# gevaertlab/RNA-GAN

Hardware: AMD Instinct MI355X
Metric: training imgs/sec (G+D WGAN-GP step, 256x256) (higher is better)
Workload: dtype bf16; 1 GPU; RNA-GAN lung (betaVAE-conditioned wganvae path) 256x256, DCGAN enc2048/step64, per-GPU batch 64, one iteration = G-loss + D-loss + GP steps; global_batch=64, parallelism=dp1, ranks=1, rna_features=19198, hip_graphs=True, dp_statistics=rank-local (DDP)

## Files before the change

rna_gan_amd/csrc/rg_api.hip:

```cpp
#include "rg_common.h"
#include "rg_internal.h"
#include <stdarg.h>
#include <stdio.h>
#include <stdlib.h>
#include <string.h>
#include <ctype.h>

static thread_local char g_err[512] = "";

void rg_set_error(const char* fmt, ...) {
  va_list ap;
  va_start(ap, fmt);
  vsnprintf(g_err, sizeof(g_err), fmt, ap);
  va_end(ap);
}

extern "C" int rg_version(void) { return 618; }
extern "C" const char* rg_last_error(void) { return g_err; }

static const char* const g_opt_names[] = {"conv8", "conv8_blocks", "conv_tile", "xcd", "class_fast", "wgrad_blocks",
                                          "wgrad8", "conv_v1", "stream_tile", "narrow8", "conv8_mfma", "conv8_epi", "wgrad8_blocks", "korder", "convp", "convp_blocks",
                                          "fp8_mx", "wgrad8n", "f32mma", "convd", "convd_blocks", "skinny128", "slab16", "wslab16", "bn_rev", "wgrad8_mfma", "narrow32", "upimg", "upimg_blocks"};
constexpr int G_NOPT = sizeof(g_opt_names) / sizeof(g_opt_names[0]);
static int g_opt_override[G_NOPT];
static int g_opt_env[G_NOPT];

int rg_option(const char* name, int dflt) {
  for (int i = 0; i < G_NOPT; ++i) {
    if (strcmp(name, g_opt_names[i]) != 0) continue;
    if (g_opt_override[i] > 0) return g_opt_override[i] - 1;
    if (g_opt_env[i] == 0) {
      char var[64] = "RNAGAN_";
      size_t n = strlen(var);
      for (const char* c = name; *c && n + 1 < sizeof(var); ++c) var[n++] = (char)toupper((unsigned char)*c);
      var[n] = 0;
      const char* e = getenv(var);
      g_opt_env[i] = e ? atoi(e) + 1 : -1;
      if (g_opt_env[i] == 0) g_opt_env[i] = -1;
    }
    return g_opt_env[i] > 0 ? g_opt_env[i] - 1 : dflt;
  }
  return dflt;
}

extern "C" int rg_set_option(const char* name, int value) {
  RG_REQUIRE(name, RG_EINVAL, "set_option: null name");
  for (int i = 0; i < G_NOPT; ++i)
    if (strcmp(name, g_opt_names[i]) == 0) { g_opt_override[i] = value < 0 ? 0 : value + 1; return RG_OK; }
  rg_set_error("set_option: unknown option '%s'", name);
  return RG_EINVAL;
}

static bool want_mfma(int algo, int dtype) { return algo != RG_ALGO_GENERIC && dtype == RG_H16; }

extern "C" int rg_pack_conv_weight(const float* w, void* wdn, void* wup, int O, int I, int dtype, void* stream) {
  RG_REQUIRE(w && O > 0 && I > 0, RG_EINVAL, "pack_conv_weight: bad args");
  RG_REQUIRE(dtype == RG_H16, RG_EUNSUPPORTED, "pack_conv_weight: only bf16 packs exist (fp32 kernels read w)");
  return rg_mfma_pack_conv_weight(w, wdn, wup, O, I, rg_stream(stream));
}

static bool conv_planned(int up, int N, int Hlow, int Wlow, int O, int I, int dtype, int algo) {
  return N > 0 && Hlow > 0 && Wlow > 0 && O > 0 && I > 0 && want_mfma(algo, dtype) &&
         rg_mfma_conv_supported(N, Hlow, Wlow, up ? O : I, up ? I : O);
}
extern "C" size_t rg_conv_workspace_bytes(int up, int N, int Hlow, int Wlow, int O, int I, int dtype, int algo) {
  return conv_planned(up, N, Hlow, Wlow, O, I, dtype, algo) ? rg_mfma_conv_plan(up, N, Hlow, Wlow, O, I).ws_bytes : 0;
}
extern "C" int rg_conv_stats_rows(int up, int N, int Hlow, int Wlow, int O, int I, int dtype, int algo) {
  return conv_planned(up, N, Hlow, Wlow, O, I, dtype, algo) ? rg_mfma_conv_plan(up, N, Hlow, Wlow, O, I).stats_rows : 0;
}
extern "C" int rg_conv_split(int up, int N, int Hlow, int Wlow, int O, int I, int dtype, int algo) {
  return conv_planned(up, N, Hlow, Wlow, O, I, dtype, algo) ? rg_mfma_conv_plan(up, N, Hlow, Wlow, O, I).nsplit : 1;
}
extern "C" int rg_conv_slab_dtype(int up, int N, int Hlow, int Wlow, int O, int I, int dtype, int algo) {
  return conv_planned(up, N, Hlow, Wlow, O, I, dtype, algo) && rg_mfma_conv_plan(up, N, Hlow, Wlow, O, I).slab16 ? RG_H16 : RG_F32;
}

extern "C" int rg_conv_down_partial(const void* x, const void* wdn, int N, int Hi, int Wi, int I, int O, int dtype, int algo,
                                    void* ws, size_t ws_bytes, void* stream) {
  RG_REQUIRE(x && wdn && ws && N > 0 && Hi > 0 && Wi > 0 && I > 0 && O > 0 && Hi % 2 == 0 && Wi % 2 == 0, RG_EINVAL,
             "conv_down_partial: bad args");
  RG_REQUIRE(rg_conv_split(0, N, Hi / 2, Wi / 2, O, I, dtype, algo) > 1, RG_EUNSUPPORTED,
             "conv_down_partial: this shape does not run split-K (rg_conv_split)");
  return rg_mfma_conv_down(x, wdn, nullptr, N, Hi, Wi, I, O, nullptr, ws, ws_bytes, rg_stream(stream), 1);
}

extern "C" int rg_conv_up_partial(const void* x, const void* wup, int N, int Ho, int Wo, int O, int I, int dtype, int algo,
                                  void* ws, size_t ws_bytes, void* stream) {
  RG_REQUIRE(x && wup && ws && N > 0 && Ho > 0 && Wo > 0 && I > 0 && O > 0, RG_EINVAL, "conv_up_partial: bad args");
  RG_REQUIRE(rg_conv_split(1, N, Ho, Wo, O, I, dtype, algo) > 1, RG_EUNSUPPORTED,
             "conv_up_partial: this shape does not run split-K (rg_conv_split)");
  return rg_mfma_conv_up(x, wup, nullptr, N, Ho, Wo, O, I, nullptr, 1.f, nullptr, ws, ws_bytes, rg_stream(stream), nullptr,
                         nullptr, 1.f, 0, 1);
}

extern "C" int rg_conv_down(const void* x, const float* w, const void* wdn, void* y, int N, int Hi, int Wi, int I,
                            int O, float* stats_partial, int dtype, int algo, void* ws, size_t ws_bytes, void* stream) {
  RG_REQUIRE(x && y && N > 0 && Hi > 0 && Wi > 0 && I > 0 && O > 0 && Hi % 2 == 0 && Wi % 2 == 0, RG_EINVAL,
             "conv_down: bad args");
  if (want_mfma(algo, dtype) && wdn && rg_mfma_conv_supported(N, Hi / 2, Wi / 2, I, O))
    return rg_mfma_conv_down(x, wdn, y, N, Hi, Wi, I, O, stats_partial, ws, ws_bytes, rg_stream(stream));
  RG_REQUIRE(!stats_partial, RG_EUNSUPPORTED, "conv_down: statistics come from the MFMA epilogue only");
  RG_REQUIRE(algo != RG_ALGO_MFMA, RG_EUNSUPPORTED, "conv_down: shape/dtype not supported by the MFMA kernel");
  RG_REQUIRE(w, RG_EINVAL, "conv_down: generic kernel needs the fp32 master weight");
  return rg_generic_conv_down(x, w, y, N, Hi, Wi, I, O, dtype, rg_stream(stream));
}

extern "C" int rg_conv_up(const void* x, const float* w, const void* wup, void* y, int N, int Ho, int Wo, int O, int I,
                          const void* mask_act, float mask_slope, float* stats_partial, int dtype, int algo, void* ws,
                          size_t ws_bytes, void* stream) {
  RG_REQUIRE(x && y && N > 0 && Ho > 0 && Wo > 0 && I > 0 && O > 0, RG_EINVAL, "conv_up: bad args");
  RG_REQUIRE(!(mask_act && stats_partial), RG_EINVAL, "conv_up: mask and statistics are exclusive");
  if (want_mfma(algo, dtype) && wup && rg_mfma_conv_supported(N, Ho, Wo, O, I))
    return rg_mfma_conv_up(x, wup, y, N, Ho, Wo, O, I, mask_act, mask_slope, stats_partial, ws, ws_bytes,
                           rg_stream(stream));
  RG_REQUIRE(!stats_partial, RG_EUNSUPPORTED, "conv_up: statistics come from the MFMA epilogue only");
  RG_REQUIRE(algo != RG_ALGO_MFMA, RG_EUNSUPPORTED, "conv_up: shape/dtype not supported by the MFMA kernel");
  RG_REQUIRE(w, RG_EINVAL, "conv_up: generic kernel needs the fp32 master weight");
  return rg_generic_conv_up(x, w, y, N, Ho, Wo, O, I, mask_act, mask_slope, dtype, rg_stream(stream));
}

extern "C" size_t rg_conv_wgrad_workspace_bytes(int N, int Ho, int Wo, int O, int I, int dtype, int algo) {
  size_t a = rg_generic_wgrad_ws_bytes(N, Ho, Wo, O, I);
  size_t b = 0;
  if (want_mfma(algo, dtype) && rg_mfma_wgrad_supported(N, Ho, Wo, O, I)) {
    b = rg_mfma_wgrad_ws_bytes(N, Ho, Wo, O, I);
    for (int two = 0; two < 2; ++two) {
      const size_t c = rg_mfma_wgrad_plan(N * Ho * Wo, two != 0, O, I).ws_bytes;
      if (c > b) b = c;
    }
  }
  return a > b ? a : b;
}

extern "C" int rg_conv_wgrad2(const void* low0, const void* high0, const void* low1, const void* high1, float* dw,
                              int N, int Ho, int Wo, int O, int I, int dtype, int accumulate, int algo, void* ws,
                              size_t ws_bytes, void* stream) {
  RG_REQUIRE(low0 && high0 && low1 && high1 && dw && N > 0 && Ho > 0 && Wo > 0 && I > 0 && O > 0, RG_EINVAL,
             "conv_wgrad2: bad args");
  if (want_mfma(algo, dtype) && rg_mfma_wgrad_supported(N, Ho, Wo, O, I))
    return rg_mfma_conv_wgrad2(low0, high0, low1, high1, dw, N, Ho, Wo, O, I, accumulate, ws, ws_bytes,
                               rg_stream(stream));
  RG_REQUIRE(algo != RG_ALGO_MFMA, RG_EUNSUPPORTED, "conv_wgrad2: shape/dtype not supported by the MFMA kernel");
  int rc = rg_generic_conv_wgrad(low0, high0, dw, N, Ho, Wo, O, I, dtype, accumulate, ws, ws_bytes, rg_stream(stream));
  if (rc) return rc;
  return rg_generic_conv_wgrad(low1, high1, dw, N, Ho, Wo, O, I, dtype, 1, ws, ws_bytes, rg_stream(stream));
}

extern "C" int rg_conv_wgrad_slabs(const void* low0, const void* high0, const void* low1, const void* high1, float* dw, int N,
                                   int Ho, int Wo, int O, int I, int dtype, int algo, void* slab, size_t slab_bytes,
                                   int* nsplit_out, int* slab_dtype_out, void* stream) {
  RG_REQUIRE(low0 && high0 && dw && nsplit_out && slab_dtype_out && (low1 == nullptr) == (high1 == nullptr) && N > 0 && Ho > 0 &&
                 Wo > 0 && I > 0 && O > 0, RG_EINVAL, "conv_wgrad_slabs: bad args");
  *slab_dtype_out = RG_F32;
  if (!(want_mfma(algo, dtype) && rg_mfma_wgrad_supported(N, Ho, Wo, O, I))) {
    *nsplit_out = 1;
    RG_REQUIRE(algo != RG_ALGO_MFMA, RG_EUNSUPPORTED, "conv_wgrad_slabs: shape/dtype not supported by the MFMA kernel");
    int rc = rg_generic_conv_wgrad(low0, high0, dw, N, Ho, Wo, O, I, dtype, 0, slab, slab_bytes, rg_stream(stream));
    if (rc || !low1) return rc;
    return rg_generic_conv_wgrad(low1, high1, dw, N, Ho, Wo, O, I, dtype, 1, slab, slab_bytes, rg_stream(stream));
  }
  return rg_mfma_conv_wgrad2(low0, high0, low1, high1, dw, N, Ho, Wo, O, I, 0, slab, slab_bytes, rg_stream(stream), nsplit_out,
                             slab_dtype_out);
}

extern "C" int rg_conv_wgrad_adam_supported(int N, int Ho, int Wo, int O, int I, int two, int dtype, int algo) {
  if (!(N > 0 && Ho > 0 && Wo > 0 && O > 0 && I > 0 && want_mfma(algo, dtype) && rg_mfma_wgrad_supported(N, Ho, Wo, O, I))) return 0;
  const RgWgradPlan pl = rg_mfma_wgrad_plan(N * Ho * Wo, two != 0, O, I);
  return pl.kernel == RG_WK_WGRAD8 && pl.nsplit == 1 ? 1 : 0;
}
extern "C" int rg_conv_wgrad_adam(const void* low0, const void* high0, const void* low1, const void* high1, float* p, float* m,
                                  float* v, const float* hyper, void* shadow_bf16, int N, int Ho, int Wo, int O, int I, int dtype,
                                  int algo, void* stream) {
  RG_REQUIRE(low0 && high0 && p && m && v && hyper && (low1 == nullptr) == (high1 == nullptr) && N > 0 && Ho > 0 && Wo > 0 &&
                 I > 0 && O > 0, RG_EINVAL, "conv_wgrad_adam: bad args");
// ... 342 lines not shown
```

rna_gan_amd/csrc/rg_splitbn.hip:

```cpp
#include "rg_internal.h"

namespace {

constexpr int SB_COLS = 128;
constexpr int SB_TY = 64;
constexpr int SB_ERR = 0;

typedef unsigned __attribute__((address_space(1))) gu32;
typedef unsigned u32x4 __attribute__((ext_vector_type(4)));

struct SbnArgs {
  const float* slab; size_t slab_stride; int nsplit;
  int slab16;
  const uint16_t* zin;
  uint16_t* out0;
  uint16_t* out1;
  int M;
  int C, groups, rbpg;
  const float* gamma; const float* beta; float slope, eps, momentum;
  float* mean; float* invstd;
  float* rmean; float* rvar; long long* nbt;
  float* s_gy; float* s_gyxh;
  float* dgamma; float* dbeta; int accumulate;
  float* part;
  unsigned* sync;
};

__device__ __forceinline__ gu32* as_global(const void* p) { return (gu32*)(unsigned*)const_cast<void*>(p); }
__device__ __forceinline__ void st_sc1(float* p, float v) {
  __hip_atomic_store(as_global(p), __float_as_uint(v), __ATOMIC_RELAXED, __HIP_MEMORY_SCOPE_AGENT);
}
__device__ __forceinline__ float ld_sc1(const float* p) {
  return __uint_as_float(__hip_atomic_load(as_global(p), __ATOMIC_RELAXED, __HIP_MEMORY_SCOPE_AGENT));
}

__device__ __forceinline__ void slice_rendezvous(unsigned* sync, int slice, unsigned members) {
  gu32* arrive = as_global(sync + 16 + 16 * slice);
  gu32* gen = arrive + 1;
  unsigned g0 = 0;
  if (threadIdx.x == 0) g0 = __hip_atomic_load(gen, __ATOMIC_RELAXED, __HIP_MEMORY_SCOPE_AGENT);
  asm volatile("s_waitcnt vmcnt(0)" ::: "memory");
  __syncthreads();
  if (threadIdx.x == 0) {
    const unsigned old = __hip_atomic_fetch_add(arrive, 1u, __ATOMIC_RELAXED, __HIP_MEMORY_SCOPE_AGENT);
    if (old == members - 1) {
      __hip_atomic_store(arrive, 0u, __ATOMIC_RELAXED, __HIP_MEMORY_SCOPE_AGENT);
      asm volatile("s_waitcnt vmcnt(0)" ::: "memory");
      __hip_atomic_fetch_add(gen, 1u, __ATOMIC_RELAXED, __HIP_MEMORY_SCOPE_AGENT);
    } else {
      unsigned spins = 0;
      while (__hip_atomic_load(gen, __ATOMIC_RELAXED, __HIP_MEMORY_SCOPE_AGENT) == g0) {
        __builtin_amdgcn_s_sleep(2);
        if (++spins > (1u << 26)) {
          __hip_atomic_store(as_global(sync + SB_ERR), 1u, __ATOMIC_RELAXED, __HIP_MEMORY_SCOPE_AGENT);
          break;
        }
      }
    }
    __builtin_amdgcn_fence(__ATOMIC_ACQUIRE, "agent");
    asm volatile("s_waitcnt vmcnt(0)" ::: "memory");
  }
  __syncthreads();
}

__device__ __forceinline__ void unpack8(const uint4& t, float* o) {
  o[0] = h16lo_to_f32(t.x); o[1] = h16hi_to_f32(t.x);
  o[2] = h16lo_to_f32(t.y); o[3] = h16hi_to_f32(t.y);
  o[4] = h16lo_to_f32(t.z); o[5] = h16hi_to_f32(t.z);
  o[6] = h16lo_to_f32(t.w); o[7] = h16hi_to_f32(t.w);
}
__device__ __forceinline__ uint4 pack8(const float* v) {
  uint4 t;
  t.x = (uint32_t)f32_to_h16(v[0]) | ((uint32_t)f32_to_h16(v[1]) << 16);
  t.y = (uint32_t)f32_to_h16(v[2]) | ((uint32_t)f32_to_h16(v[3]) << 16);
  t.z = (uint32_t)f32_to_h16(v[4]) | ((uint32_t)f32_to_h16(v[5]) << 16);
  t.w = (uint32_t)f32_to_h16(v[6]) | ((uint32_t)f32_to_h16(v[7]) << 16);
  return t;
}

template <int NS, bool S16> struct SlabPiece;
template <int NS> struct SlabPiece<NS, false> { float4 v[NS][2]; };
template <int NS> struct SlabPiece<NS, true> { uint4 v[NS]; };
template <int NS>
__device__ __forceinline__ void slab_load(const float* __restrict__ p, size_t off, size_t stride, SlabPiece<NS, false>& q) {
#pragma unroll
  for (int s = 0; s < NS; ++s) {
    q.v[s][0] = *reinterpret_cast<const float4*>(p + off + s * stride);
    q.v[s][1] = *reinterpret_cast<const float4*>(p + off + s * stride + 4);
  }
}
template <int NS>
__device__ __forceinline__ void slab_load(const float* __restrict__ p, size_t off, size_t stride, SlabPiece<NS, true>& q) {
  const uint16_t* h = reinterpret_cast<const uint16_t*>(p);
#pragma unroll
  for (int s = 0; s < NS; ++s) q.v[s] = *reinterpret_cast<const uint4*>(h + off + s * stride);
}
template <int NS>
__device__ __forceinline__ void slab_sum(const SlabPiece<NS, false>& q, float* acc) {
#pragma unroll
  for (int i = 0; i < 8; ++i) acc[i] = 0.f;
#pragma unroll
  for (int s = 0; s < NS; ++s) {
    acc[0] += q.v[s][0].x; acc[1] += q.v[s][0].y; acc[2] += q.v[s][0].z; acc[3] += q.v[s][0].w;
    acc[4] += q.v[s][1].x; acc[5] += q.v[s][1].y; acc[6] += q.v[s][1].z; acc[7] += q.v[s][1].w;
  }
}
template <int NS>
__device__ __forceinline__ void slab_sum(const SlabPiece<NS, true>& q, float* acc) {
#pragma unroll
  for (int i = 0; i < 8; ++i) acc[i] = 0.f;
#pragma unroll
  for (int s = 0; s < NS; ++s) {
    float v[8];
    unpack8(q.v[s], v);
#pragma unroll
    for (int i = 0; i < 8; ++i) acc[i] += v[i];
  }
}

constexpr int SB_THREADS = 1024;
constexpr int SB_WAVES = SB_THREADS / 64;

__device__ __forceinline__ void block_partial(float (*sm)[2][SB_COLS], float* s1, float* s2, float* prow) {
  const int lane = threadIdx.x & 63, wave = threadIdx.x >> 6, tx = lane & 15;
#pragma unroll
  for (int i = 0; i < 8; ++i) {
    s1[i] += __shfl_xor(s1[i], 16, 64); s1[i] += __shfl_xor(s1[i], 32, 64);
    s2[i] += __shfl_xor(s2[i], 16, 64); s2[i] += __shfl_xor(s2[i], 32, 64);
  }
  if (lane < 16) {
#pragma unroll
    for (int i = 0; i < 8; ++i) { sm[wave][0][tx * 8 + i] = s1[i]; sm[wave][1][tx * 8 + i] = s2[i]; }
  }
  __syncthreads();
  if (threadIdx.x < 2 * SB_COLS) {
    const int q = threadIdx.x / SB_COLS, col = threadIdx.x % SB_COLS;
    float t = 0.f;
#pragma unroll
    for (int k = 0; k < SB_WAVES; ++k) t += sm[k][q][col];
    st_sc1(prow + q * SB_COLS + col, t);
  }
}

__device__ __forceinline__ void slice_totals(const float* pgrp, int rbpg, float (*lanes)[2 * SB_COLS], float* tot) {
  const int q4 = threadIdx.x & 63, rl = threadIdx.x >> 6;
  const __amdgpu_buffer_rsrc_t rs = __builtin_amdgcn_make_buffer_rsrc((void*)pgrp, 0, rbpg * 2 * SB_COLS * 4, 0x00020000);
  float4 acc = make_float4(0.f, 0.f, 0.f, 0.f);
  u32x4 v[4];
#pragma unroll
  for (int k = 0; k < 4; ++k) {
    const int r = rl + 16 * k;
    v[k] = __builtin_amdgcn_raw_buffer_load_b128(rs, r < rbpg ? (r * 2 * SB_COLS + q4 * 4) * 4 : 0x7ffffff0, 0, 16);
  }
#pragma unroll
  for (int k = 0; k < 4; ++k) {
    acc.x += __uint_as_float(v[k].x); acc.y += __uint_as_float(v[k].y);
    acc.z += __uint_as_float(v[k].z); acc.w += __uint_as_float(v[k].w);
  }
  *reinterpret_cast<float4*>(&lanes[rl][q4 * 4]) = acc;
  __syncthreads();
  if (threadIdx.x < 2 * SB_COLS) {
    float t = 0.f;
#pragma unroll
    for (int k = 0; k < SB_WAVES; ++k) t += lanes[k][threadIdx.x];
    tot[threadIdx.x] = t;
  }
  __syncthreads();
}

template <int RPT, int NS, bool S16>
__global__ __launch_bounds__(SB_THREADS) void slab_bn_fwd_kernel(SbnArgs a) {
  __shared__ __attribute__((aligned(16))) float sm[SB_WAVES][2][SB_COLS];
  __shared__ float tot[2 * SB_COLS];
  float (*lanes)[2 * SB_COLS] = reinterpret_cast<float (*)[2 * SB_COLS]>(&sm[0][0][0]);
  const int tx = threadIdx.x % 16, ty = threadIdx.x / 16;
  const int slice = blockIdx.x, grp = blockIdx.y / a.rbpg, rb = blockIdx.y - grp * a.rbpg;
  const int c = slice * SB_COLS + tx * 8;
  const size_t row0 = (size_t)grp * a.M + (size_t)rb * (RPT * SB_TY) + ty;
  uint4 zp[RPT];
  float s1[8], s2[8];
#pragma unroll
  for (int i = 0; i < 8; ++i) { s1[i] = 0.f; s2[i] = 0.f; }
  constexpr int U = (8 / NS) < RPT ? (8 / NS) : RPT;
#pragma unroll
  for (int k0 = 0; k0 < RPT; k0 += U) {
    SlabPiece<NS, S16> q[U];
#pragma unroll
    for (int u = 0; u < U; ++u) slab_load<NS>(a.slab, (row0 + (size_t)(k0 + u) * SB_TY) * a.C + c, a.slab_stride, q[u]);
#pragma unroll
    for (int u = 0; u < U; ++u) {
      const int k = k0 + u;
      float acc[8];
      slab_sum<NS>(q[u], acc);
      zp[k] = pack8(acc);
      *reinterpret_cast<uint4*>(a.out0 + (row0 + (size_t)k * SB_TY) * a.C + c) = zp[k];
      float v[8];
      unpack8(zp[k], v);
#pragma unroll
      for (int i = 0; i < 8; ++i) { s1[i] += v[i]; s2[i] += v[i] * v[i]; }
    }
  }
  float* pslice = a.part + (size_t)slice * a.groups * a.rbpg * 2 * SB_COLS;
  block_partial(sm, s1, s2, pslice + ((size_t)grp * a.rbpg + rb) * 2 * SB_COLS);
  slice_rendezvous(a.sync, slice, (unsigned)(a.groups * a.rbpg));

  const float m = (float)a.M;
  if (rb == 0 && grp == 0) {
    const int col = threadIdx.x % SB_COLS;
    float rm = 0.f, rv = 0.f;
    if (a.rmean && threadIdx.x < SB_COLS) { rm = a.rmean[slice * SB_COLS + col]; rv = a.rvar[slice * SB_COLS + col]; }
    for (int g = 0; g < a.groups; ++g) {
      slice_totals(pslice + (size_t)g * a.rbpg * 2 * SB_COLS, a.rbpg, lanes, tot);
      if (threadIdx.x < SB_COLS) {
        const double mud = (double)tot[col] / (double)m;
        const float mu = (float)mud;
        const float var = (float)fmax((double)tot[SB_COLS + col] / (double)m - mud * mud, 0.0);
        a.mean[(size_t)g * a.C + slice * SB_COLS + col] = mu;
        a.invstd[(size_t)g * a.C + slice * SB_COLS + col] = rsqrtf(var + a.eps);
        if (a.rmean) {
          const float unb = var * (m / fmaxf(m - 1.f, 1.f));
          rm = (1.f - a.momentum) * rm + a.momentum * mu;
          rv = (1.f - a.momentum) * rv + a.momentum * unb;
        }
      }
      __syncthreads();
    }
    if (a.rmean && threadIdx.x < SB_COLS) { a.rmean[slice * SB_COLS + col] = rm; a.rvar[slice * SB_COLS + col] = rv; }
    if (a.nbt && slice == 0 && threadIdx.x == 0) *a.nbt += a.groups;
  }
  if (!(rb == 0 && grp == 0 && a.groups == 1))
    slice_totals(pslice + (size_t)grp * a.rbpg * 2 * SB_COLS, a.rbpg, lanes, tot);

  float sc[8], sh[8], bet[8];
#pragma unroll
  for (int i = 0; i < 8; ++i) {
    const double mud = (double)tot[tx * 8 + i] / (double)m;
    const float mu = (float)mud;
    const float var = (float)fmax((double)tot[SB_COLS + tx * 8 + i] / (double)m - mud * mud, 0.0);
    const float rstd = rsqrtf(var + a.eps);
    sc[i] = rstd * a.gamma[c + i];
    sh[i] = mu;
    bet[i] = a.beta[c + i];
  }
#pragma unroll
  for (int k = 0; k < RPT; ++k) {
    float v[8], o[8];
    unpack8(zp[k], v);
#pragma unroll
    for (int i = 0; i < 8; ++i) o[i] = lrelu_f((v[i] - sh[i]) * sc[i] + bet[i], a.slope);
    *reinterpret_cast<uint4*>(a.out1 + (row0 + (size_t)k * SB_TY) * a.C + c) = pack8(o);
  }
}

template <int RPT, int NS, int MODE, bool S16>
__global__ __launch_bounds__(SB_THREADS) void slab_bn_bwd_kernel(SbnArgs a) {
  __shared__ __attribute__((aligned(16))) float sm[SB_WAVES][2][SB_COLS];
  __shared__ float tot[2 * SB_COLS];
  float (*lanes)[2 * SB_COLS] = reinterpret_cast<float (*)[2 * SB_COLS]>(&sm[0][0][0]);
  const int tx = threadIdx.x % 16, ty = threadIdx.x / 16;
  const int slice = blockIdx.x, grp = blockIdx.y / a.rbpg, rb = blockIdx.y - grp * a.rbpg;
  const int c = slice * SB_COLS + tx * 8;
  const size_t row0 = (size_t)grp * a.M + (size_t)rb * (RPT * SB_TY) + ty;
  float mu[8], rstd[8], gam[8], bet[8];
#pragma unroll
  for (int i = 0; i < 8; ++i) {
    mu[i] = a.mean[(size_t)grp * a.C + c + i]; rstd[i] = a.invstd[(size_t)grp * a.C + c + i];
    gam[i] = a.gamma[c + i]; bet[i] = a.beta[c + i];
  }
  uint4 gp[RPT], zp[RPT];
  float s1[8], s2[8];
#pragma unroll
  for (int i = 0; i < 8; ++i) { s1[i] = 0.f; s2[i] = 0.f; }
  constexpr int U = (8 / NS) < RPT ? (8 / NS) : RPT;
#pragma unroll
  for (int k0 = 0; k0 < RPT; k0 += U) {
    SlabPiece<NS, S16> q[U];
#pragma unroll
    for (int u = 0; u < U; ++u) {
      const size_t off = (row0 + (size_t)(k0 + u) * SB_TY) * a.C + c;
      zp[k0 + u] = *reinterpret_cast<const uint4*>(a.zin + off);
      slab_load<NS>(a.slab, off, a.slab_stride, q[u]);
    }
#pragma unroll
    for (int u = 0; u < U; ++u) {
      const int k = k0 + u;
      float acc[8];
      slab_sum<NS>(q[u], acc);
      gp[k] = pack8(acc);
      if (a.out0) *reinterpret_cast<uint4*>(a.out0 + (row0 + (size_t)k * SB_TY) * a.C + c) = gp[k];
      float g[8], v[8];
      unpack8(gp[k], g); unpack8(zp[k], v);
#pragma unroll
      for (int i = 0; i < 8; ++i) {
        const float xh = (v[i] - mu[i]) * rstd[i];
        if (MODE == 0) {
          const float gy = g[i] * lrelu_mask(xh * gam[i] + bet[i], a.slope);
          s1[i] += gy; s2[i] += gy * xh;
        } else {
          s1[i] += g[i]; s2[i] += xh * g[i];
        }
      }
    }
  }
  float* pslice = a.part + (size_t)slice * a.groups * a.rbpg * 2 * SB_COLS;
  block_partial(sm, s1, s2, pslice + ((size_t)grp * a.rbpg + rb) * 2 * SB_COLS);
  slice_rendezvous(a.sync, slice, (unsigned)(a.groups * a.rbpg));

  if (rb == 0 && grp == 0) {
    const int col = threadIdx.x % SB_COLS;
    float dg = 0.f, db = 0.f;
    for (int g = 0; g < a.groups; ++g) {
      slice_totals(pslice + (size_t)g * a.rbpg * 2 * SB_COLS, a.rbpg, lanes, tot);
      if (threadIdx.x < SB_COLS) {
        const size_t o = (size_t)g * a.C + slice * SB_COLS + col;
        a.s_gy[o] = tot[col]; a.s_gyxh[o] = tot[SB_COLS + col];
        if (g == 0) { dg = tot[SB_COLS + col]; db = tot[col]; } else { dg += tot[SB_COLS + col]; db += tot[col]; }
      }
      __syncthreads();
    }
    if (MODE == 0 && a.dgamma && threadIdx.x < SB_COLS) {
      const int o = slice * SB_COLS + col;
      if (a.accumulate) { a.dgamma[o] += dg; a.dbeta[o] += db; } else { a.dgamma[o] = dg; a.dbeta[o] = db; }
    }
  }
  if (!(rb == 0 && grp == 0 && a.groups == 1))
    slice_totals(pslice + (size_t)grp * a.rbpg * 2 * SB_COLS, a.rbpg, lanes, tot);

  const float inv_m = 1.f / (float)a.M;
  float m1[8], m2[8];
#pragma unroll
  for (int i = 0; i < 8; ++i) { m1[i] = tot[tx * 8 + i] * inv_m; m2[i] = tot[SB_COLS + tx * 8 + i] * inv_m; }
#pragma unroll
  for (int k = 0; k < RPT; ++k) {
    float g[8], v[8], o[8];
    unpack8(gp[k], g); unpack8(zp[k], v);
#pragma unroll
    for (int i = 0; i < 8; ++i) {
      const float xh = (v[i] - mu[i]) * rstd[i];
      const float mk = lrelu_mask(xh * gam[i] + bet[i], a.slope);
      if (MODE == 0) {
        const float gy = g[i] * mk;
        o[i] = (gam[i] * rstd[i]) * (gy - m1[i] - xh * m2[i]);
      } else {
        o[i] = (gam[i] * rstd[i]) * (g[i] - m1[i] - xh * m2[i]) * mk;
      }
    }
    *reinterpret_cast<uint4*>(a.out1 + (row0 + (size_t)k * SB_TY) * a.C + c) = pack8(o);
  }
}

struct SbnPlan { int rpt, rbpg, slices; };

static bool sbn_plan(int M, int C, int groups, int nsplit, SbnPlan* p) {
  if (C % SB_COLS || M <= 0 || groups < 1 || groups > 2) return false;
  if (nsplit != 2 && nsplit != 4 && nsplit != 8) return false;
  const int slices = C / SB_COLS;
  const long long rows = (long long)M * groups;
  int best = 0;
  for (int rpt = 1; rpt <= 4 && !best; rpt *= 2) {
    const int rpb = rpt * SB_TY;
    if (M % rpb || M / rpb > 64) continue;
    if (rpt * nsplit > 8) continue;
    if (rows / rpb * slices <= 256) best = rpt;
  }
  if (!best) return false;
  p->rpt = best; p->rbpg = M / (best * SB_TY); p->slices = slices;
  return true;
}

template <int KIND, int RPT>
static void sbn_launch_ns(const SbnArgs& a, dim3 grid, hipStream_t st) {
#define SBN_GO(NS)                                                                                          \
  do {                                                                                                      \
    if (KIND == 0) {                                                                                         \
      if (a.slab16) hipLaunchKernelGGL((slab_bn_fwd_kernel<RPT, NS, true>), grid, dim3(SB_THREADS), 0, st, a);  \
      else hipLaunchKernelGGL((slab_bn_fwd_kernel<RPT, NS, false>), grid, dim3(SB_THREADS), 0, st, a);          \
    } else if (a.slab16) {                                                                                   \
      hipLaunchKernelGGL((slab_bn_bwd_kernel<RPT, NS, KIND == 2 ? 1 : 0, true>), grid, dim3(SB_THREADS), 0, st, a);  \
    } else {                                                                                                 \
      hipLaunchKernelGGL((slab_bn_bwd_kernel<RPT, NS, KIND == 2 ? 1 : 0, false>), grid, dim3(SB_THREADS), 0, st, a); \
    }                                                                                                        \
  } while (0)
  if constexpr (RPT == 1) { if (a.nsplit == 2) SBN_GO(2); else if (a.nsplit == 4) SBN_GO(4); else SBN_GO(8); }
  else if constexpr (RPT == 2) { if (a.nsplit == 2) SBN_GO(2); else SBN_GO(4); }
  else SBN_GO(2);
#undef SBN_GO
}

template <int KIND>
static int sbn_launch(const char* name, SbnArgs& a, const SbnPlan& p, hipStream_t st) {
  a.rbpg = p.rbpg;
  dim3 grid((unsigned)p.slices, (unsigned)(a.groups * p.rbpg));
  switch (p.rpt) {
    case 1: sbn_launch_ns<KIND, 1>(a, grid, st); break;
    case 2: sbn_launch_ns<KIND, 2>(a, grid, st); break;
    default: sbn_launch_ns<KIND, 4>(a, grid, st); break;
  }
  RG_LAUNCH_CHECK(name);
  return RG_OK;
}

}

extern "C" int rg_slab_bn_supported(long long M, int C, int groups, int nsplit) {
  SbnPlan p;
  return M < (1ll << 30) && sbn_plan((int)M, C, groups, nsplit, &p) ? 1 : 0;
}
extern "C" size_t rg_slab_bn_scratch_bytes(long long M, int C, int groups) {
  return (size_t)((M * groups + 63) / 64) * (size_t)C * 2 * sizeof(float);
}
extern "C" size_t rg_slab_bn_sync_words(void) { return 16 + 16 * 64; }

extern "C" int rg_bn_forward_slabs(const void* slab, int nsplit, size_t slab_stride, int slab_dtype, void* z, void* a_out, long long M, int C,
                                   int groups, float eps, float momentum, const float* gamma, const float* beta, float slope,
                                   float* mean, float* invstd, float* running_mean, float* running_var,
                                   long long* num_batches_tracked, void* scratch, size_t scratch_bytes, void* sync,
                                   void* stream) {
  RG_REQUIRE(slab && z && a_out && gamma && beta && mean && invstd && scratch && sync, RG_EINVAL, "bn_forward_slabs: null");
  SbnPlan p;
  RG_REQUIRE(M < (1ll << 30) && sbn_plan((int)M, C, groups, nsplit, &p), RG_EUNSUPPORTED,
             "bn_forward_slabs: M=%lld C=%d groups=%d nsplit=%d has no fused form (rg_slab_bn_supported)", M, C, groups, nsplit);
  RG_REQUIRE(p.slices <= 64, RG_EUNSUPPORTED, "bn_forward_slabs: C > 8192");
  RG_REQUIRE(scratch_bytes >= (size_t)p.slices * groups * p.rbpg * 2 * SB_COLS * sizeof(float), RG_EWORKSPACE,
             "bn_forward_slabs: scratch too small");
  SbnArgs a{};
  a.slab = (const float*)slab; a.slab_stride = slab_stride; a.nsplit = nsplit; a.slab16 = slab_dtype == RG_H16 ? 1 : 0;
  a.out0 = (uint16_t*)z; a.out1 = (uint16_t*)a_out; a.M = (int)M; a.C = C; a.groups = groups;
  a.gamma = gamma; a.beta = beta; a.slope = slope; a.eps = eps; a.momentum = momentum;
  a.mean = mean; a.invstd = invstd; a.rmean = running_mean; a.rvar = running_var; a.nbt = num_batches_tracked;
  a.part = (float*)scratch; a.sync = (unsigned*)sync;
  return sbn_launch<0>("bn_forward_slabs", a, p, rg_stream(stream));
}

extern "C" int rg_bn_act_bwd_slabs(const void* slab, int nsplit, size_t slab_stride, int slab_dtype, const void* z, void* ga_out, void* gz,
                                   long long M, int C, int groups, const float* mean, const float* invstd, const float* gamma,
                                   const float* beta, float slope, float* s_gy, float* s_gyxh, float* dgamma, float* dbeta,
                                   int accumulate, void* scratch, size_t scratch_bytes, void* sync, void* stream) {
  RG_REQUIRE(slab && z && gz && mean && invstd && gamma && beta && s_gy && s_gyxh && scratch && sync, RG_EINVAL,
             "bn_act_bwd_slabs: null");
  RG_REQUIRE((dgamma == nullptr) == (dbeta == nullptr), RG_EINVAL, "bn_act_bwd_slabs: dgamma and dbeta go together");
  SbnPlan p;
  RG_REQUIRE(M < (1ll << 30) && sbn_plan((int)M, C, groups, nsplit, &p), RG_EUNSUPPORTED,
             "bn_act_bwd_slabs: M=%lld C=%d groups=%d nsplit=%d has no fused form (rg_slab_bn_supported)", M, C, groups, nsplit);
  RG_REQUIRE(p.slices <= 64, RG_EUNSUPPORTED, "bn_act_bwd_slabs: C > 8192");
  RG_REQUIRE(scratch_bytes >= (size_t)p.slices * groups * p.rbpg * 2 * SB_COLS * sizeof(float), RG_EWORKSPACE,
             "bn_act_bwd_slabs: scratch too small");
  SbnArgs a{};
  a.slab = (const float*)slab; a.slab_stride = slab_stride; a.nsplit = nsplit; a.slab16 = slab_dtype == RG_H16 ? 1 : 0;
  a.zin = (const uint16_t*)z; a.out0 = (uint16_t*)ga_out; a.out1 = (uint16_t*)gz; a.M = (int)M; a.C = C; a.groups = groups;
  a.gamma = gamma; a.beta = beta; a.slope = slope;
  a.mean = const_cast<float*>(mean); a.invstd = const_cast<float*>(invstd);
  a.s_gy = s_gy; a.s_gyxh = s_gyxh; a.dgamma = dgamma; a.dbeta = dbeta; a.accumulate = accumulate;
  a.part = (float*)scratch; a.sync = (unsigned*)sync;
  return sbn_launch<1>("bn_act_bwd_slabs", a, p, rg_stream(stream));
}

extern "C" int rg_bn_tangent_slabs(const void* slab, int nsplit, size_t slab_stride, int slab_dtype, const void* z, void* zt_out, void* at,
                                   long long M, int C, const float* mean, const float* invstd, const float* gamma,
                                   const float* beta, float slope, float* s_zt, float* s_xhzt, void* scratch,
                                   size_t scratch_bytes, void* sync, void* stream) {
  RG_REQUIRE(slab && z && zt_out && at && mean && invstd && gamma && beta && s_zt && s_xhzt && scratch && sync, RG_EINVAL,
             "bn_tangent_slabs: null");
  SbnPlan p;
  RG_REQUIRE(M < (1ll << 30) && sbn_plan((int)M, C, 1, nsplit, &p), RG_EUNSUPPORTED,
             "bn_tangent_slabs: M=%lld C=%d nsplit=%d has no fused form (rg_slab_bn_supported)", M, C, nsplit);
  RG_REQUIRE(p.slices <= 64, RG_EUNSUPPORTED, "bn_tangent_slabs: C > 8192");
  RG_REQUIRE(scratch_bytes >= (size_t)p.slices * p.rbpg * 2 * SB_COLS * sizeof(float), RG_EWORKSPACE,
             "bn_tangent_slabs: scratch too small");
  SbnArgs a{};
  a.slab = (const float*)slab; a.slab_stride = slab_stride; a.nsplit = nsplit; a.slab16 = slab_dtype == RG_H16 ? 1 : 0;
  a.zin = (const uint16_t*)z; a.out0 = (uint16_t*)zt_out; a.out1 = (uint16_t*)at; a.M = (int)M; a.C = C; a.groups = 1;
  a.gamma = gamma; a.beta = beta; a.slope = slope;
  a.mean = const_cast<float*>(mean); a.invstd = const_cast<float*>(invstd);
  a.s_gy = s_zt; a.s_gyxh = s_xhzt;
  a.part = (float*)scratch; a.sync = (unsigned*)sync;
  return sbn_launch<2>("bn_tangent_slabs", a, p, rg_stream(stream));
}
```

Before: 6056 imgs/sec.

## Overlap split-BN slab stores with slice rendezvous and use buffer loads

Adds a PIPE variant of the split-batchnorm forward and backward kernels, on by default. The slice barrier is split into arrive and wait phases so the out0 stores from waves other than wave 0 are issued while blocks wait on the rendezvous; wave 0 stores its out0 data later alongside out1. Loads and stores now use buffer resource descriptors with scalar offsets, and gamma, beta, mean and invstd are loaded as vectors early. The aim is to hide store and sync latency in these grid-synchronised kernels, at the cost of more live registers and extra template instantiations.

```diff
diff --git a/rna_gan_amd/csrc/rg_api.hip b/rna_gan_amd/csrc/rg_api.hip
--- a/rna_gan_amd/csrc/rg_api.hip
+++ b/rna_gan_amd/csrc/rg_api.hip
@@ -20,7 +20,7 @@
 
 static const char* const g_opt_names[] = {"conv8", "conv8_blocks", "conv_tile", "xcd", "class_fast", "wgrad_blocks",
                                           "wgrad8", "conv_v1", "stream_tile", "narrow8", "conv8_mfma", "conv8_epi", "wgrad8_blocks", "korder", "convp", "convp_blocks",
-                                          "fp8_mx", "wgrad8n", "f32mma", "convd", "convd_blocks", "skinny128", "slab16", "wslab16", "bn_rev", "wgrad8_mfma", "narrow32", "upimg", "upimg_blocks"};
+                                          "fp8_mx", "wgrad8n", "f32mma", "convd", "convd_blocks", "skinny128", "slab16", "wslab16", "bn_rev", "wgrad8_mfma", "narrow32", "upimg", "upimg_blocks", "sbn_pipe"};
 constexpr int G_NOPT = sizeof(g_opt_names) / sizeof(g_opt_names[0]);
 static int g_opt_override[G_NOPT];
 static int g_opt_env[G_NOPT];
diff --git a/rna_gan_amd/csrc/rg_splitbn.hip b/rna_gan_amd/csrc/rg_splitbn.hip
--- a/rna_gan_amd/csrc/rg_splitbn.hip
+++ b/rna_gan_amd/csrc/rg_splitbn.hip
@@ -63,12 +63,50 @@
   __syncthreads();
 }
 
+struct SliceTicket { unsigned g0; bool last; };
+__device__ __forceinline__ SliceTicket slice_arrive(unsigned* sync, int slice, unsigned members) {
+  gu32* arrive = as_global(sync + 16 + 16 * slice);
+  gu32* gen = arrive + 1;
+  SliceTicket t{0u, false};
+  if (threadIdx.x == 0) t.g0 = __hip_atomic_load(gen, __ATOMIC_RELAXED, __HIP_MEMORY_SCOPE_AGENT);
+  asm volatile("s_waitcnt vmcnt(0)" ::: "memory");
+  __syncthreads();
+  if (threadIdx.x == 0) {
+    const unsigned old = __hip_atomic_fetch_add(arrive, 1u, __ATOMIC_RELAXED, __HIP_MEMORY_SCOPE_AGENT);
+    t.last = old == members - 1;
+    if (t.last) {
+      __hip_atomic_store(arrive, 0u, __ATOMIC_RELAXED, __HIP_MEMORY_SCOPE_AGENT);
+      asm volatile("s_waitcnt vmcnt(0)" ::: "memory");
+      __hip_atomic_fetch_add(gen, 1u, __ATOMIC_RELAXED, __HIP_MEMORY_SCOPE_AGENT);
+    }
+  }
+  return t;
+}
+__device__ __forceinline__ void slice_wait(unsigned* sync, int slice, const SliceTicket& t) {
+  if (threadIdx.x == 0) {
+    if (!t.last) {
+      gu32* gen = as_global(sync + 16 + 16 * slice) + 1;
+      unsigned spins = 0;
+      while (__hip_atomic_load(gen, __ATOMIC_RELAXED, __HIP_MEMORY_SCOPE_AGENT) == t.g0) {
+        __builtin_amdgcn_s_sleep(2);
+        if (++spins > (1u << 26)) {
+          __hip_atomic_store(as_global(sync + SB_ERR), 1u, __ATOMIC_RELAXED, __HIP_MEMORY_SCOPE_AGENT);
+          break;
+        }
+      }
+    }
+    __builtin_amdgcn_fence(__ATOMIC_ACQUIRE, "agent");
+  }
+  __syncthreads();
+}
+
 __device__ __forceinline__ void unpack8(const uint4& t, float* o) {
   o[0] = h16lo_to_f32(t.x); o[1] = h16hi_to_f32(t.x);
   o[2] = h16lo_to_f32(t.y); o[3] = h16hi_to_f32(t.y);
   o[4] = h16lo_to_f32(t.z); o[5] = h16hi_to_f32(t.z);
   o[6] = h16lo_to_f32(t.w); o[7] = h16hi_to_f32(t.w);
 }
+__device__ __forceinline__ void keep_packed(uint4& t) { asm volatile("" : "+v"(t.x), "+v"(t.y), "+v"(t.z), "+v"(t.w)); }
 __device__ __forceinline__ uint4 pack8(const float* v) {
   uint4 t;
   t.x = (uint32_t)f32_to_h16(v[0]) | ((uint32_t)f32_to_h16(v[1]) << 16);
@@ -78,6 +116,12 @@
   return t;
 }
 
+typedef float f32x4u __attribute__((ext_vector_type(4), aligned(4)));
+__device__ __forceinline__ void param8(const float* p, float* o) {
+  const f32x4u lo = *reinterpret_cast<const f32x4u*>(p), hi = *reinterpret_cast<const f32x4u*>(p + 4);
+  o[0] = lo.x; o[1] = lo.y; o[2] = lo.z; o[3] = lo.w; o[4] = hi.x; o[5] = hi.y; o[6] = hi.z; o[7] = hi.w;
+}
+
 template <int NS, bool S16> struct SlabPiece;
 template <int NS> struct SlabPiece<NS, false> { float4 v[NS][2]; };
 template <int NS> struct SlabPiece<NS, true> { uint4 v[NS]; };
@@ -95,6 +139,36 @@
 #pragma unroll
   for (int s = 0; s < NS; ++s) q.v[s] = *reinterpret_cast<const uint4*>(h + off + s * stride);
 }
+typedef __amdgpu_buffer_rsrc_t brsrc;
+__device__ __forceinline__ brsrc blk_rsrc(const void* base, unsigned nrec) {
+  return __builtin_amdgcn_make_buffer_rsrc(const_cast<void*>(base), 0, (int)nrec, 0x00020000);
+}
+__device__ __forceinline__ uint4 ld_b128(brsrc rs, unsigned voff, unsigned soff) {
+  const u32x4 v = __builtin_amdgcn_raw_buffer_load_b128(rs, (int)voff, (int)soff, 0);
+  return make_uint4(v.x, v.y, v.z, v.w);
+}
+__device__ __forceinline__ void st_b128(brsrc rs, unsigned voff, unsigned soff, const uint4& t) {
+  u32x4 v; v.x = t.x; v.y = t.y; v.z = t.z; v.w = t.w;
+  __builtin_amdgcn_raw_buffer_store_b128(v, rs, (int)voff, (int)soff, 0);
+}
+template <int NS>
+__device__ __forceinline__ void slab_load_b(const float* p, size_t ublk, unsigned nrec16, unsigned t16, unsigned soff16, size_t stride,
+                                            SlabPiece<NS, false>& q) {
+#pragma unroll
+  for (int s = 0; s < NS; ++s) {
+    const brsrc rs = blk_rsrc(p + ublk + s * stride, nrec16 * 2u);
+    const uint4 lo = ld_b128(rs, t16 * 2u, soff16 * 2u), hi = ld_b128(rs, t16 * 2u + 16u, soff16 * 2u);
+    q.v[s][0] = make_float4(__uint_as_float(lo.x), __uint_as_float(lo.y), __uint_as_float(lo.z), __uint_as_float(lo.w));
+    q.v[s][1] = make_float4(__uint_as_float(hi.x), __uint_as_float(hi.y), __uint_as_float(hi.z), __uint_as_float(hi.w));
+  }
+}
+template <int NS>
+__device__ __forceinline__ void slab_load_b(const float* p, size_t ublk, unsigned nrec16, unsigned t16, unsigned soff16, size_t stride,
+                                            SlabPiece<NS, true>& q) {
+  const uint16_t* h = reinterpret_cast<const uint16_t*>(p);
+#pragma unroll
+  for (int s = 0; s < NS; ++s) q.v[s] = ld_b128(blk_rsrc(h + ublk + s * stride, nrec16), t16, soff16);
+}
 template <int NS>
 __device__ __forceinline__ void slab_sum(const SlabPiece<NS, false>& q, float* acc) {
 #pragma unroll
@@ -168,7 +242,7 @@
   __syncthreads();
 }
 
-template <int RPT, int NS, bool S16>
+template <int RPT, int NS, bool S16, bool PIPE>
 __global__ __launch_bounds__(SB_THREADS) void slab_bn_fwd_kernel(SbnArgs a) {
   __shared__ __attribute__((aligned(16))) float sm[SB_WAVES][2][SB_COLS];
   __shared__ float tot[2 * SB_COLS];
@@ -177,8 +251,23 @@
   const int slice = blockIdx.x, grp = blockIdx.y / a.rbpg, rb = blockIdx.y - grp * a.rbpg;
   const int c = slice * SB_COLS + tx * 8;
   const size_t row0 = (size_t)grp * a.M + (size_t)rb * (RPT * SB_TY) + ty;
+  const size_t blk = ((size_t)grp * a.M + (size_t)rb * (RPT * SB_TY)) * a.C + (size_t)slice * SB_COLS;
+  const unsigned nrec16 = ((unsigned)(RPT * SB_TY - 1) * (unsigned)a.C + SB_COLS) * 2u, rstep16 = (unsigned)SB_TY * (unsigned)a.C * 2u;
+  const unsigned t16 = ((unsigned)ty * (unsigned)a.C + (unsigned)tx * 8u) * 2u;
+  [[maybe_unused]] auto ld16 = [&](const uint16_t* p, int k) -> uint4 {
+    if constexpr (PIPE) return ld_b128(blk_rsrc(p + blk, nrec16), t16, (unsigned)k * rstep16);
+    else return *reinterpret_cast<const uint4*>(p + (row0 + (size_t)k * SB_TY) * a.C + c);
+  };
+  auto st16 = [&](uint16_t* p, int k, const uint4& v) {
+    if constexpr (PIPE) st_b128(blk_rsrc(p + blk, nrec16), t16, (unsigned)k * rstep16, v);
+    else *reinterpret_cast<uint4*>(p + (row0 + (size_t)k * SB_TY) * a.C + c) = v;
+  };
+  auto slabs = [&](int k, SlabPiece<NS, S16>& q) {
+    if constexpr (PIPE) slab_load_b<NS>(a.slab, blk, nrec16, t16, (unsigned)k * rstep16, a.slab_stride, q);
+    else slab_load<NS>(a.slab, (row0 + (size_t)k * SB_TY) * a.C + c, a.slab_stride, q);
+  };
   uint4 zp[RPT];
-  float s1[8], s2[8];
+  float s1[8], s2[8], gam[8], bet[8];
 #pragma unroll
   for (int i = 0; i < 8; ++i) { s1[i] = 0.f; s2[i] = 0.f; }
   constexpr int U = (8 / NS) < RPT ? (8 / NS) : RPT;
@@ -186,14 +275,15 @@
   for (int k0 = 0; k0 < RPT; k0 += U) {
     SlabPiece<NS, S16> q[U];
 #pragma unroll
-    for (int u = 0; u < U; ++u) slab_load<NS>(a.slab, (row0 + (size_t)(k0 + u) * SB_TY) * a.C + c, a.slab_stride, q[u]);
+    for (int u = 0; u < U; ++u) slabs(k0 + u, q[u]);
+    if (PIPE && k0 == 0) { param8(a.gamma + c, gam); param8(a.beta + c, bet); }
 #pragma unroll
     for (int u = 0; u < U; ++u) {
       const int k = k0 + u;
       float acc[8];
       slab_sum<NS>(q[u], acc);
       zp[k] = pack8(acc);
-      *reinterpret_cast<uint4*>(a.out0 + (row0 + (size_t)k * SB_TY) * a.C + c) = zp[k];
+      if (!PIPE) st16(a.out0, k, zp[k]);
       float v[8];
       unpack8(zp[k], v);
 #pragma unroll
@@ -202,7 +292,17 @@
   }
   float* pslice = a.part + (size_t)slice * a.groups * a.rbpg * 2 * SB_COLS;
   block_partial(sm, s1, s2, pslice + ((size_t)grp * a.rbpg + rb) * 2 * SB_COLS);
-  slice_rendezvous(a.sync, slice, (unsigned)(a.groups * a.rbpg));
+  const bool wave0 = threadIdx.x < 64;
+  if (PIPE) {
+    const SliceTicket tk = slice_arrive(a.sync, slice, (unsigned)(a.groups * a.rbpg));
+    if (!wave0) {
+#pragma unroll
+      for (int k = 0; k < RPT; ++k) st16(a.out0, k, zp[k]);
+    }
+    slice_wait(a.sync, slice, tk);
+  } else {
+    slice_rendezvous(a.sync, slice, (unsigned)(a.groups * a.rbpg));
+  }
 
   const float m = (float)a.M;
   if (rb == 0 && grp == 0) {
@@ -231,16 +331,16 @@
   if (!(rb == 0 && grp == 0 && a.groups == 1))
     slice_totals(pslice + (size_t)grp * a.rbpg * 2 * SB_COLS, a.rbpg, lanes, tot);
 
-  float sc[8], sh[8], bet[8];
+  float sc[8], sh[8];
 #pragma unroll
   for (int i = 0; i < 8; ++i) {
     const double mud = (double)tot[tx * 8 + i] / (double)m;
     const float mu = (float)mud;
     const float var = (float)fmax((double)tot[SB_COLS + tx * 8 + i] / (double)m - mud * mud, 0.0);
     const float rstd = rsqrtf(var + a.eps);
-    sc[i] = rstd * a.gamma[c + i];
+    if (!PIPE) { gam[i] = a.gamma[c + i]; bet[i] = a.beta[c + i]; }
+    sc[i] = rstd * gam[i];
     sh[i] = mu;
-    bet[i] = a.beta[c + i];
   }
 #pragma unroll
   for (int k = 0; k < RPT; ++k) {
@@ -248,11 +348,12 @@
     unpack8(zp[k], v);
 #pragma unroll
     for (int i = 0; i < 8; ++i) o[i] = lrelu_f((v[i] - sh[i]) * sc[i] + bet[i], a.slope);
-    *reinterpret_cast<uint4*>(a.out1 + (row0 + (size_t)k * SB_TY) * a.C + c) = pack8(o);
-  }
-}
-
-template <int RPT, int NS, int MODE, bool S16>
+    if (PIPE && wave0) st16(a.out0, k, zp[k]);
+    st16(a.out1, k, pack8(o));
+  }
+}
+
+template <int RPT, int NS, int MODE, bool S16, bool PIPE>
 __global__ __launch_bounds__(SB_THREADS) void slab_bn_bwd_kernel(SbnArgs a) {
   __shared__ __attribute__((aligned(16))) float sm[SB_WAVES][2][SB_COLS];
   __shared__ float tot[2 * SB_COLS];
@@ -261,11 +362,28 @@
   const int slice = blockIdx.x, grp = blockIdx.y / a.rbpg, rb = blockIdx.y - grp * a.rbpg;
   const int c = slice * SB_COLS + tx * 8;
   const size_t row0 = (size_t)grp * a.M + (size_t)rb * (RPT * SB_TY) + ty;
+  const size_t blk = ((size_t)grp * a.M + (size_t)rb * (RPT * SB_TY)) * a.C + (size_t)slice * SB_COLS;
+  const unsigned nrec16 = ((unsigned)(RPT * SB_TY - 1) * (unsigned)a.C + SB_COLS) * 2u, rstep16 = (unsigned)SB_TY * (unsigned)a.C * 2u;
+  const unsigned t16 = ((unsigned)ty * (unsigned)a.C + (unsigned)tx * 8u) * 2u;
+  [[maybe_unused]] auto ld16 = [&](const uint16_t* p, int k) -> uint4 {
+    if constexpr (PIPE) return ld_b128(blk_rsrc(p + blk, nrec16), t16, (unsigned)k * rstep16);
+    else return *reinterpret_cast<const uint4*>(p + (row0 + (size_t)k * SB_TY) * a.C + c);
+  };
+  auto st16 = [&](uint16_t* p, int k, const uint4& v) {
+    if constexpr (PIPE) st_b128(blk_rsrc(p + blk, nrec16), t16, (unsigned)k * rstep16, v);
+    else *reinterpret_cast<uint4*>(p + (row0 + (size_t)k * SB_TY) * a.C + c) = v;
+  };
+  auto slabs = [&](int k, SlabPiece<NS, S16>& q) {
+    if constexpr (PIPE) slab_load_b<NS>(a.slab, blk, nrec16, t16, (unsigned)k * rstep16, a.slab_stride, q);
+    else slab_load<NS>(a.slab, (row0 + (size_t)k * SB_TY) * a.C + c, a.slab_stride, q);
+  };
   float mu[8], rstd[8], gam[8], bet[8];
-#pragma unroll
-  for (int i = 0; i < 8; ++i) {
-    mu[i] = a.mean[(size_t)grp * a.C + c + i]; rstd[i] = a.invstd[(size_t)grp * a.C + c + i];
-    gam[i] = a.gamma[c + i]; bet[i] = a.beta[c + i];
+  if (!PIPE) {
+#pragma unroll
+    for (int i = 0; i < 8; ++i) {
+      mu[i] = a.mean[(size_t)grp * a.C + c + i]; rstd[i] = a.invstd[(size_t)grp * a.C + c + i];
+      gam[i] = a.gamma[c + i]; bet[i] = a.beta[c + i];
+    }
   }
   uint4 gp[RPT], zp[RPT];
   float s1[8], s2[8];
@@ -277,9 +395,12 @@
     SlabPiece<NS, S16> q[U];
 #pragma unroll
     for (int u = 0; u < U; ++u) {
-      const size_t off = (row0 + (size_t)(k0 + u) * SB_TY) * a.C + c;
-      zp[k0 + u] = *reinterpret_cast<const uint4*>(a.zin + off);
-      slab_load<NS>(a.slab, off, a.slab_stride, q[u]);
+      zp[k0 + u] = ld16(a.zin, k0 + u);
+      slabs(k0 + u, q[u]);
+    }
+    if (PIPE && k0 == 0) {
+      param8(a.mean + (size_t)grp * a.C + c, mu); param8(a.invstd + (size_t)grp * a.C + c, rstd);
+      param8(a.gamma + c, gam); param8(a.beta + c, bet);
     }
 #pragma unroll
     for (int u = 0; u < U; ++u) {
@@ -287,7 +408,7 @@
       float acc[8];
       slab_sum<NS>(q[u], acc);
       gp[k] = pack8(acc);
-      if (a.out0) *reinterpret_cast<uint4*>(a.out0 + (row0 + (size_t)k * SB_TY) * a.C + c) = gp[k];
+      if (!PIPE && a.out0) st16(a.out0, k, gp[k]);
       float g[8], v[8];
       unpack8(gp[k], g); unpack8(zp[k], v);
 #pragma unroll
@@ -304,7 +425,19 @@
   }
   float* pslice = a.part + (size_t)slice * a.groups * a.rbpg * 2 * SB_COLS;
   block_partial(sm, s1, s2, pslice + ((size_t)grp * a.rbpg + rb) * 2 * SB_COLS);
-  slice_rendezvous(a.sync, slice, (unsigned)(a.groups * a.rbpg));
+  const bool wave0 = threadIdx.x < 64;
+  if (PIPE) {
+    const SliceTicket tk = slice_arrive(a.sync, slice, (unsigned)(a.groups * a.rbpg));
+    if (!wave0 && a.out0) {
+#pragma unroll
+      for (int k = 0; k < RPT; ++k) st16(a.out0, k, gp[k]);
+    }
+    slice_wait(a.sync, slice, tk);
+#pragma unroll
+    for (int k = 0; k < RPT; ++k) { keep_packed(gp[k]); keep_packed(zp[k]); }
+  } else {
+    slice_rendezvous(a.sync, slice, (unsigned)(a.groups * a.rbpg));
+  }
 
   if (rb == 0 && grp == 0) {
     const int col = threadIdx.x % SB_COLS;
@@ -345,7 +478,8 @@
         o[i] = (gam[i] * rstd[i]) * (g[i] - m1[i] - xh * m2[i]) * mk;
       }
     }
-    *reinterpret_cast<uint4*>(a.out1 + (row0 + (size_t)k * SB_TY) * a.C + c) = pack8(o);
+    if (PIPE && wave0 && a.out0) st16(a.out0, k, gp[k]);
+    st16(a.out1, k, pack8(o));
   }
 }
 
@@ -368,18 +502,19 @@
   return true;
 }
 
+template <int KIND, int RPT, int NS, bool S16, bool PIPE>
+static void sbn_go(const SbnArgs& a, dim3 grid, hipStream_t st) {
+  if constexpr (KIND == 0) hipLaunchKernelGGL((slab_bn_fwd_kernel<RPT, NS, S16, PIPE>), grid, dim3(SB_THREADS), 0, st, a);
+  else hipLaunchKernelGGL((slab_bn_bwd_kernel<RPT, NS, KIND == 2 ? 1 : 0, S16, PIPE>), grid, dim3(SB_THREADS), 0, st, a);
+}
+
 template <int KIND, int RPT>
 static void sbn_launch_ns(const SbnArgs& a, dim3 grid, hipStream_t st) {
+  const bool pipe = rg_option("sbn_pipe", 1) != 0;
 #define SBN_GO(NS)                                                                                          \
   do {                                                                                                      \
-    if (KIND == 0) {                                                                                         \
-      if (a.slab16) hipLaunchKernelGGL((slab_bn_fwd_kernel<RPT, NS, true>), grid, dim3(SB_THREADS), 0, st, a);  \
-      else hipLaunchKernelGGL((slab_bn_fwd_kernel<RPT, NS, false>), grid, dim3(SB_THREADS), 0, st, a);          \
-    } else if (a.slab16) {                                                                                   \
-      hipLaunchKernelGGL((slab_bn_bwd_kernel<RPT, NS, KIND == 2 ? 1 : 0, true>), grid, dim3(SB_THREADS), 0, st, a);  \
-    } else {                                                                                                 \
-      hipLaunchKernelGGL((slab_bn_bwd_kernel<RPT, NS, KIND == 2 ? 1 : 0, false>), grid, dim3(SB_THREADS), 0, st, a); \
-    }                                                                                                        \
+    if (a.slab16) { if (pipe) sbn_go<KIND, RPT, NS, true, true>(a, grid, st); else sbn_go<KIND, RPT, NS, true, false>(a, grid, st); }    \
+    else { if (pipe) sbn_go<KIND, RPT, NS, false, true>(a, grid, st); else sbn_go<KIND, RPT, NS, false, false>(a, grid, st); }          \
   } while (0)
   if constexpr (RPT == 1) { if (a.nsplit == 2) SBN_GO(2); else if (a.nsplit == 4) SBN_GO(4); else SBN_GO(8); }
   else if constexpr (RPT == 2) { if (a.nsplit == 2) SBN_GO(2); else SBN_GO(4); }
```

New measurement: 6093 imgs/sec, median of 3. About the same (+0.6%).
